# wkvong/multimodal-baby

Measured on AMD Instinct MI355X. Metric: image-text pairs/sec, CVCL ResNeXt+embed 224², bs256, 1/2/4/8 MI355X, higher is better.
Workload: dtype bf16; 1 GPU; C2 = BASELINE configs[1]: CVCL saycam_contrastive, frozen random-init ResNeXt-50 32x4d (BN train mode) + embedding mean-pool text encoder, E=512, L2-normalised, fixed tau 0.07, 224x224 frames + 3-word utterances; full step = fwd + InfoNCE + bwd(fc, embedding) + AdamW; per_gpu_batch=256, global_batch=256, negatives=local (single GPU), parallelism=dp1, trunk_streams=2

## Files before the change

multimodal-baby_amd/csrc/resnext.hip:

```cpp
#include <algorithm>
#include <array>
#include <cstdlib>
#include <type_traits>

#include "cvcl_common.h"

namespace {

constexpr int kMaxStatsRows = 1024;
constexpr size_t kTrunkAccLayer = (size_t)kBnAccRows * 2 * 2048;


__global__ __launch_bounds__(1024) void bn_finalize_kernel(const float* __restrict__ stats, int rows, double count,
                                                           const float* __restrict__ gamma, const float* __restrict__ beta,
                                                           float* __restrict__ running_mean, float* __restrict__ running_var,
                                                           int64_t* __restrict__ nbt, float momentum, float eps,
                                                           float* __restrict__ scale, float* __restrict__ shift, int C,
                                                           float* __restrict__ moments, int moments_ld,
                                                           const float* __restrict__ centre) {
    constexpr int NS = 64, NC = 16;
    __shared__ double ps[NS][NC], pq[NS][NC];
    const int c = threadIdx.x & (NC - 1), sl = threadIdx.x / NC, ch = blockIdx.x * NC + c;
    double s = 0.0, q = 0.0;
    if (ch < C) {
// ... 96 lines not shown
            q = fmaf(v, v, q);
        }
    }
    ps[sl][c] = s;
    pq[sl][c] = q;
    __syncthreads();
    if (sl == 0 && ch < C) {
        stats[((long)blockIdx.x * 2 + 0) * C + ch] = (ps[0][c] + ps[1][c]) + (ps[2][c] + ps[3][c]);
        stats[((long)blockIdx.x * 2 + 1) * C + ch] = (pq[0][c] + pq[1][c]) + (pq[2][c] + pq[3][c]);
    }
}

template <typename T>
__global__ void cast_kernel(const float* __restrict__ in, T* __restrict__ out, long n) {
    for (long i = (long)blockIdx.x * blockDim.x + threadIdx.x; i < n; i += (long)gridDim.x * blockDim.x)
        out[i] = ElemTraits<T>::from_f(in[i]);
}

__global__ void pack_stem_kernel(const float* __restrict__ w, bf16_t* __restrict__ out) {
    const int i = blockIdx.x * blockDim.x + threadIdx.x;
    if (i >= 4 * 6 * 16 * 32) return;
    const int k = i & 31, n = (i >> 5) & 15, ks = (i >> 9) % 6, nt = i / (6 * 512);
    const int r = 4 * ks + (k >> 3), kx = k & 7;
    float v = 0.f;
    if (r < 21 && kx < 7) {
        const int c = r / 7, ky = r % 7;
        v = w[((nt * 16 + n) * 3 + c) * 49 + ky * 7 + kx];
    }
    out[i] = (bf16_t)v;
}

__global__ void pack_gconv_kernel(const float* __restrict__ w, bf16_t* __restrict__ out, int C, int cg) {
    const int KS = cg == 32 ? 9 : 5;
    const long total = (long)(C / 16) * KS * 512;
    const long i = (long)blockIdx.x * blockDim.x + threadIdx.x;
    if (i >= total) return;
    const int k = (int)(i & 31), n = (int)((i >> 5) & 15), ks = (int)((i >> 9) % KS), unit = (int)(i / ((long)KS * 512));
    const int co = unit * 16 + n;
    float v = 0.f;
    if (cg == 32) {
        v = w[((long)co * 32 + k) * 9 + ks];
    } else {
        const int tap = 2 * ks + (k >> 4), ci_abs = unit * 16 + (k & 15);
        if (tap < 9 && ci_abs / cg == co / cg) v = w[((long)co * cg + (ci_abs % cg)) * 9 + tap];
    }
    out[i] = (bf16_t)v;
}

constexpr int STEM_TH = 4;
constexpr int STEM_ROWS = 2 * STEM_TH + 5;
constexpr int STEM_PITCH = 144;
constexpr int STEM_OPITCH = 144;

__global__ __launch_bounds__(256, 2) void stem_mfma_kernel(const float* __restrict__ x, const bf16_t* __restrict__ wp,
                                                        bf16_t* __restrict__ y, float* __restrict__ stats,
                                                        const float* __restrict__ centre, int B, int Hin, int Win) {
    extern __shared__ __attribute__((aligned(16))) char smem[];
    unsigned int* patch = (unsigned int*)smem;
    const int Ho = Hin / 2, Wo = Win / 2;
    const int bands = cvcl_div_up(Ho, STEM_TH);
    const int tid = threadIdx.x, lane = tid & 63, wave = tid >> 6;
    const int pix = lane & 15, kb = lane >> 4;

    bf16x8 wf[4][6];
#pragma unroll
    for (int nt = 0; nt < 4; ++nt)
#pragma unroll
        for (int ks = 0; ks < 6; ++ks)
            wf[nt][ks] = *reinterpret_cast<const bf16x8*>(wp + ((nt * 6 + ks) * 16 + pix) * 32 + kb * 8);

    f32x2 ssum[4][2], ssq[4][2];
#pragma unroll
    for (int a = 0; a < 4; ++a)
#pragma unroll
        for (int b = 0; b < 2; ++b) { ssum[a][b] = f32x2{0.f, 0.f}; ssq[a][b] = f32x2{0.f, 0.f}; }

    const int mtiles_per_row = cvcl_div_up(Wo, 16);
    const int wave_u = __builtin_amdgcn_readfirstlane(wave);
    int koff[6];
#pragma unroll
    for (int ks = 0; ks < 6; ++ks) {
        const int r = min(4 * ks + kb, 20);
        const int c = r / 7, ky = r - c * 7;
        koff[ks] = (c * STEM_ROWS + ky) * STEM_PITCH;
    }
    for (int i = tid; i < 3 * STEM_ROWS * STEM_PITCH; i += 256) patch[i] = 0u;
    char* wst = smem + 3 * STEM_ROWS * STEM_PITCH * 4 + wave * (16 * STEM_OPITCH);
    float* cen = reinterpret_cast<float*>(smem + 3 * STEM_ROWS * STEM_PITCH * 4 + 4 * 16 * STEM_OPITCH);
    if (tid < 64) cen[tid] = centre ? -centre[tid] : 0.f;
    const int bx = (gridDim.x & 7) == 0 ? (int)((blockIdx.x & 7) * (gridDim.x >> 3) + (blockIdx.x >> 3)) : (int)blockIdx.x;
    for (int item = bx; item < B * bands; item += gridDim.x) {
        const int b = item / bands, band = item - b * bands;
        const int oy0 = band * STEM_TH;
        __syncthreads();
        {
            constexpr int NROW = 3 * STEM_ROWS, NV = 5;
            const int vec_per_row = Win / 4, jl = min(lane, vec_per_row - 1);
#pragma unroll
            for (int half = 0; half < 2; ++half) {
                f32x4 v[NV];
#pragma unroll
                for (int i = 0; i < NV; ++i) {
                    const int r = min((half * NV + i) * 4 + wave_u, NROW - 1);
                    const int c = r / STEM_ROWS, iy = r - c * STEM_ROWS;
                    const int yin = min(max(2 * oy0 - 3 + iy, 0), Hin - 1);
                    v[i] = *reinterpret_cast<const f32x4*>(x + (((long)b * 3 + c) * Hin + yin) * Win + 4 * jl);
                }
#pragma unroll
                for (int i = 0; i < NV; ++i) {
                    const int r = (half * NV + i) * 4 + wave_u;
                    const int iy = r % STEM_ROWS, yin = 2 * oy0 - 3 + iy;
                    if (r < NROW && lane < vec_per_row) {
                        const bool ok = yin >= 0 && yin < Hin;
                        const unsigned u01 = ok ? round2(f32x2{v[i][0], v[i][1]}) : 0u, u23 = ok ? round2(f32x2{v[i][2], v[i][3]}) : 0u;
                        char* dst = reinterpret_cast<char*>(patch + r * STEM_PITCH) + 8 * lane + 6;
                        *reinterpret_cast<unsigned short*>(dst) = (unsigned short)u01;
                        *reinterpret_cast<unsigned*>(dst + 2) = (u01 >> 16) | (u23 << 16);
                        *reinterpret_cast<unsigned short*>(dst + 6) = (unsigned short)(u23 >> 16);
                    }
                }
            }
        }
        __syncthreads();
        int ty = 0, tx = wave_u;
        while (tx >= mtiles_per_row) { tx -= mtiles_per_row; ++ty; }
        while (ty < STEM_TH) {
            const int ox0 = tx * 16;
            const int oy = oy0 + ty, ox = ox0 + pix;
            f32x4 acc[4];
#pragma unroll
            for (int nt = 0; nt < 4; ++nt) acc[nt] = *reinterpret_cast<const f32x4*>(cen + nt * 16 + kb * 4);
            const unsigned int* row0 = patch + 2 * ty * STEM_PITCH + (ox < Wo ? ox : 0);
#pragma unroll
            for (int ks = 0; ks < 6; ++ks) {
                const unsigned int* src = row0 + koff[ks];
                u32x4 raw = {src[0], src[1], src[2], src[3]};
                const bf16x8 bfrag = __builtin_bit_cast(bf16x8, raw);
#pragma unroll
                for (int nt = 0; nt < 4; ++nt)
                    acc[nt] = __builtin_amdgcn_mfma_f32_16x16x32_bf16(wf[nt][ks], bfrag, acc[nt], 0, 0, 0);
            }
            const bool inside = oy < Ho && ox < Wo;
#pragma unroll
            for (int nt = 0; nt < 4; ++nt) {
                const u32x2 o = {round2(f32x2{acc[nt][0], acc[nt][1]}), round2(f32x2{acc[nt][2], acc[nt][3]})};
                *reinterpret_cast<u32x2*>(wst + pix * STEM_OPITCH + nt * 32 + kb * 8) = o;
                if (inside) {
#pragma unroll
                    for (int e = 0; e < 2; ++e) {
                        const f32x2 sv = widen2(o[e]);
                        ssum[nt][e] += sv;
                        ssq[nt][e] = __builtin_elementwise_fma(sv, sv, ssq[nt][e]);
                    }
                }
            }
            __builtin_amdgcn_wave_barrier();
            asm volatile("" ::: "memory");
            if (oy < Ho && y) {
                bf16_t* drow = y + (((long)b * Ho + oy) * Wo + ox0) * 64 + (lane & 7) * 8;
#pragma unroll
                for (int rd = 0; rd < 2; ++rd) {
                    const int px = (lane >> 3) + 8 * rd;
                    const u32x4 v = *reinterpret_cast<const u32x4*>(wst + px * STEM_OPITCH + (lane & 7) * 16);
                    if (ox0 + px < Wo) *reinterpret_cast<u32x4*>(drow + (long)px * 64) = v;
                }
            }
            __builtin_amdgcn_wave_barrier();
            asm volatile("" ::: "memory");
            tx += 4;
            while (tx >= mtiles_per_row) { tx -= mtiles_per_row; ++ty; }
        }
    }
    __syncthreads();
    float* red = (float*)smem;
#pragma unroll
    for (int nt = 0; nt < 4; ++nt)
#pragma unroll
        for (int e = 0; e < 4; ++e) {
            float s = ssum[nt][e >> 1][e & 1], q = ssq[nt][e >> 1][e & 1];
#pragma unroll
            for (int o = 1; o < 16; o <<= 1) { s += __shfl_xor(s, o, 64); q += __shfl_xor(q, o, 64); }
            if (pix == 0) {
                red[(wave * 2 + 0) * 64 + nt * 16 + kb * 4 + e] = s;
                red[(wave * 2 + 1) * 64 + nt * 16 + kb * 4 + e] = q;
            }
        }
    __syncthreads();
    if (tid < 128) {
        const int which = tid >> 6, c = tid & 63;
        const float v = (red[(0 * 2 + which) * 64 + c] + red[(1 * 2 + which) * 64 + c]) +
                        (red[(2 * 2 + which) * 64 + c] + red[(3 * 2 + which) * 64 + c]);
        stats[((long)blockIdx.x * 2 + which) * 64 + c] = v;
    }
}

constexpr int STEMP_TP = 2;
constexpr int STEMP_CR = 2 * STEMP_TP + 1;
constexpr int STEMP_ROWS = 2 * STEMP_CR + 5;
constexpr int STEMP_BW = 128;
constexpr int STEMP_BAND_BYTES = (STEMP_CR * STEMP_BW + 1) * 128;
__global__ __launch_bounds__(512, 1) void stem_pool_mfma_kernel(const float* __restrict__ x, const bf16_t* __restrict__ wp,
                                                                bf16_t* __restrict__ y, const float* __restrict__ scale,
                                                                const float* __restrict__ shift, const float* __restrict__ centre,
                                                                int B, int Hin, int Win) {
    extern __shared__ __attribute__((aligned(16))) char smem[];
    unsigned int* patch = (unsigned int*)smem;
    char* band = smem + 3 * STEMP_ROWS * STEM_PITCH * 4;
    float* cen = reinterpret_cast<float*>(band + STEMP_BAND_BYTES);
    const int Ho = Hin / 2, Wo = Win / 2;
    const int Hp = (Ho - 1) / 2 + 1, Wp = (Wo - 1) / 2 + 1;
    const int bands = cvcl_div_up(Hp, STEMP_TP);
    const int tid = threadIdx.x, lane = tid & 63;
    const int wave_u = __builtin_amdgcn_readfirstlane(tid >> 6);
    const int pix = lane & 15, kb = lane >> 4;

    bf16x8 wf[4][6];
#pragma unroll
    for (int nt = 0; nt < 4; ++nt)
#pragma unroll
        for (int ks = 0; ks < 6; ++ks)
            wf[nt][ks] = *reinterpret_cast<const bf16x8*>(wp + ((nt * 6 + ks) * 16 + pix) * 32 + kb * 8);
    const int mtiles_per_row = cvcl_div_up(Wo, 16);
    int koff[6];
#pragma unroll
    for (int ks = 0; ks < 6; ++ks) {
        const int r = min(4 * ks + kb, 20);
        const int c = r / 7, ky = r - c * 7;
        koff[ks] = (c * STEMP_ROWS + ky) * STEM_PITCH;
    }
    for (int i = tid; i < 3 * STEMP_ROWS * STEM_PITCH; i += 512) patch[i] = 0u;
    for (int i = tid; i < STEMP_CR * STEMP_BW * 32; i += 512) reinterpret_cast<unsigned*>(band)[i] = 0u;
    if (tid < 64) {
        cen[tid] = centre ? -centre[tid] : 0.f;
        cen[64 + tid] = scale[tid];
        cen[128 + tid] = shift[tid];
    }
    const int bx = (gridDim.x & 7) == 0 ? (int)((blockIdx.x & 7) * (gridDim.x >> 3) + (blockIdx.x >> 3)) : (int)blockIdx.x;
    for (int item = bx; item < B * bands; item += gridDim.x) {
        const int b = item / bands, bnd = item - b * bands;
        const int p0 = bnd * STEMP_TP;
        const int oy_first = 2 * p0 - 1;
        {
            constexpr int NROW = 3 * STEMP_ROWS, NV = (NROW + 15) / 16;
            const int vec_per_row = Win / 4, jl = min(lane, vec_per_row - 1);
#pragma unroll
            for (int half = 0; half < 2; ++half) {
                f32x4 v[NV];
#pragma unroll
                for (int i = 0; i < NV; ++i) {
                    const int r = min((half * NV + i) * 8 + wave_u, NROW - 1);
                    const int c = r / STEMP_ROWS, iy = r - c * STEMP_ROWS;
                    const int yin = min(max(2 * oy_first - 3 + iy, 0), Hin - 1);
                    v[i] = *reinterpret_cast<const f32x4*>(x + (((long)b * 3 + c) * Hin + yin) * Win + 4 * jl);
                }
#pragma unroll
                for (int i = 0; i < NV; ++i) {
                    const int r = (half * NV + i) * 8 + wave_u;
                    const int iy = r % STEMP_ROWS, yin = 2 * oy_first - 3 + iy;
                    if (r < NROW && lane < vec_per_row) {
                        const bool ok = yin >= 0 && yin < Hin;
                        const unsigned u01 = ok ? round2(f32x2{v[i][0], v[i][1]}) : 0u, u23 = ok ? round2(f32x2{v[i][2], v[i][3]}) : 0u;
                        char* dst = reinterpret_cast<char*>(patch + r * STEM_PITCH) + 8 * lane + 6;
                        *reinterpret_cast<unsigned short*>(dst) = (unsigned short)u01;
                        *reinterpret_cast<unsigned*>(dst + 2) = (u01 >> 16) | (u23 << 16);
                        *reinterpret_cast<unsigned short*>(dst + 6) = (unsigned short)(u23 >> 16);
                    }
                }
            }
        }
        __syncthreads();
        for (int t = wave_u; t < STEMP_CR * mtiles_per_row; t += 8) {
            const int ty = t / mtiles_per_row, tx = t - ty * mtiles_per_row;
            const int ox0 = tx * 16, ox = ox0 + pix;
            const int oy = oy_first + ty;
            char* brow = band + (ty * STEMP_BW + ox + 1) * 128 + kb * 8;
            if (oy < 0 || oy >= Ho) {
#pragma unroll
                for (int nt = 0; nt < 4; ++nt) *reinterpret_cast<u32x2*>(brow + nt * 32) = u32x2{0u, 0u};
                continue;
            }
            f32x4 acc[4];
#pragma unroll
            for (int nt = 0; nt < 4; ++nt) acc[nt] = *reinterpret_cast<const f32x4*>(cen + nt * 16 + kb * 4);
            const unsigned int* row0 = patch + 2 * ty * STEM_PITCH + (ox < Wo ? ox : 0);
#pragma unroll
            for (int ks = 0; ks < 6; ++ks) {
                const unsigned int* src = row0 + koff[ks];
                u32x4 raw = {src[0], src[1], src[2], src[3]};
                const bf16x8 bfrag = __builtin_bit_cast(bf16x8, raw);
#pragma unroll
                for (int nt = 0; nt < 4; ++nt)
                    acc[nt] = __builtin_amdgcn_mfma_f32_16x16x32_bf16(wf[nt][ks], bfrag, acc[nt], 0, 0, 0);
            }
            const bool inside = ox < Wo;
#pragma unroll
            for (int nt = 0; nt < 4; ++nt) {
                const u32x2 o = {round2(f32x2{acc[nt][0], acc[nt][1]}), round2(f32x2{acc[nt][2], acc[nt][3]})};
                const f32x4 sc4 = *reinterpret_cast<const f32x4*>(cen + 64 + nt * 16 + kb * 4);
                const f32x4 sh4 = *reinterpret_cast<const f32x4*>(cen + 128 + nt * 16 + kb * 4);
                const f32x2 r01 = widen2(o[0]), r23 = widen2(o[1]);
                const f32x2 v01 = {fmaxf(fmaf(r01[0], sc4[0], sh4[0]), 0.f), fmaxf(fmaf(r01[1], sc4[1], sh4[1]), 0.f)};
                const f32x2 v23 = {fmaxf(fmaf(r23[0], sc4[2], sh4[2]), 0.f), fmaxf(fmaf(r23[1], sc4[3], sh4[3]), 0.f)};
                *reinterpret_cast<u32x2*>(brow + nt * 32) = inside ? u32x2{round2(v01), round2(v23)} : u32x2{0u, 0u};
            }
        }
        __syncthreads();
        typedef unsigned short u16x8 __attribute__((ext_vector_type(8)));
        for (int u = tid; u < STEMP_TP * Wp * 8; u += 512) {
            const int c8 = u & 7, q = u >> 3;
            const int pr = q / Wp, pc = q - pr * Wp;
            if (p0 + pr >= Hp) continue;
            const char* src = band + ((2 * pr) * STEMP_BW + 2 * pc) * 128 + c8 * 16;
            u16x8 m = *reinterpret_cast<const u16x8*>(src);
#pragma unroll
            for (int dy = 0; dy < 3; ++dy)
#pragma unroll
                for (int dx = 0; dx < 3; ++dx) {
                    if (dy == 0 && dx == 0) continue;
                    m = __builtin_elementwise_max(m, *reinterpret_cast<const u16x8*>(src + (dy * STEMP_BW + dx) * 128));
                }
            *reinterpret_cast<u16x8*>(y + (((long)b * Hp + p0 + pr) * Wp + pc) * 64 + c8 * 8) = m;
        }
    }
}

__global__ __launch_bounds__(256) void stem_direct_f32_kernel(const float* __restrict__ x, const float* __restrict__ w,
                                                              float* __restrict__ y, const float* __restrict__ centre,
                                                              int B, int Hin, int Win) {
    const int Ho = Hin / 2, Wo = Win / 2;
    const long total = (long)B * Ho * Wo * 64;
    for (long i = (long)blockIdx.x * blockDim.x + threadIdx.x; i < total; i += (long)gridDim.x * blockDim.x) {
        const int co = (int)(i & 63);
        const long p = i >> 6;
        const int ox = (int)(p % Wo), oy = (int)((p / Wo) % Ho), b = (int)(p / ((long)Wo * Ho));
        float acc = centre ? -centre[co] : 0.f;
        for (int c = 0; c < 3; ++c)
            for (int ky = 0; ky < 7; ++ky) {
                const int yin = 2 * oy - 3 + ky;
                if (yin < 0 || yin >= Hin) continue;
                for (int kx = 0; kx < 7; ++kx) {
                    const int xin = 2 * ox - 3 + kx;
                    if (xin < 0 || xin >= Win) continue;
                    acc = fmaf(x[(((long)b * 3 + c) * Hin + yin) * Win + xin], w[((co * 3 + c) * 7 + ky) * 7 + kx], acc);
                }
            }
        y[i] = acc;
    }
}

__global__ __launch_bounds__(256) void stem_tiled_f32_kernel(const float* __restrict__ x, const float* __restrict__ w,
                                                             float* __restrict__ y, const float* __restrict__ centre,
                                                             int B, int Hin, int Win, int TH, int bands) {
    extern __shared__ __attribute__((aligned(16))) float smf[];
    const int Ho = Hin / 2, Wo = Win / 2;
    const int Wp = Win + 6, rows_in = 2 * TH + 5, plane = rows_in * Wp;
    float* ws = smf;
    float* cs = ws + 147 * 64;
    float* xs = cs + 64;
    const int tid = threadIdx.x, lane = tid & 63;
    const int wave = __builtin_amdgcn_readfirstlane(tid >> 6);
    for (int e = tid; e < 147 * 64; e += 256) {
        const int co = e / 147, tap = e - co * 147;
        ws[tap * 64 + co] = w[e];
    }
    if (tid < 64) cs[tid] = centre ? -centre[tid] : 0.f;
    for (int item = blockIdx.x; item < B * bands; item += gridDim.x) {
        const int b = item / bands, band = item - b * bands;
        const int oy0 = band * TH, iy0 = 2 * oy0 - 3;
        __syncthreads();
        for (int e = tid; e < 3 * plane; e += 256) {
            const int c = e / plane, r = e - c * plane, ry = r / Wp, rx = r - ry * Wp;
            const int yin = iy0 + ry, xin = rx - 3;
// ... 700 lines not shown
        if (kind == CVCL_PACK_GCONV3) {
            CVCL_CHECK_ARG(k == 3, "cvcl_pack_conv_weight: grouped conv must be 3x3");
            return cvcl_pack_split_conv(0, w_oihw, out, cout, cin_per_group, stream);
        }
        cvcl_set_error("cvcl_pack_conv_weight: unknown kind %d", kind);
        return CVCL_EINVAL;
    }
    if (dtype == CVCL_F32) {
        hipLaunchKernelGGL(cast_kernel<float>, dim3(cvcl_grid(n, 256, 4096)), dim3(256), 0, s, w_oihw, (float*)out, n);
    } else if (kind == CVCL_PACK_DENSE) {
        hipLaunchKernelGGL(cast_kernel<bf16_t>, dim3(cvcl_grid(n, 256, 4096)), dim3(256), 0, s, w_oihw, (bf16_t*)out, n);
    } else if (kind == CVCL_PACK_STEM7) {
        CVCL_CHECK_ARG(cout == 64 && cin_per_group == 3 && k == 7, "cvcl_pack_conv_weight: stem must be 64x3x7x7");
        hipLaunchKernelGGL(pack_stem_kernel, dim3(cvcl_div_up(4 * 6 * 512, 256)), dim3(256), 0, s, w_oihw, (bf16_t*)out);
    } else if (kind == CVCL_PACK_GCONV3) {
        CVCL_CHECK_ARG(k == 3 && (cin_per_group == 4 || cin_per_group == 8 || cin_per_group == 16 || cin_per_group == 32) &&
                           cout % 64 == 0, "cvcl_pack_conv_weight: unsupported grouped conv %d/%d", cout, cin_per_group);
        const long total = (long)(cout / 16) * (cin_per_group == 32 ? 9 : 5) * 512;
        hipLaunchKernelGGL(pack_gconv_kernel, dim3(cvcl_div_up(total, 256)), dim3(256), 0, s, w_oihw, (bf16_t*)out, cout,
                           cin_per_group);
    } else {
        cvcl_set_error("cvcl_pack_conv_weight: unknown kind %d", kind);
        return CVCL_EINVAL;
    }
    CVCL_LAUNCH_CHECK();
    return CVCL_OK;
}

static int stem_grid(int B, int Hin) {
    const int items = B * cvcl_div_up(Hin / 2, STEM_TH);
    return items < 512 ? items : 512;
}

extern "C" int cvcl_stem_conv_stats_rows(int dtype, int B, int H, int W) {
    if (!cvcl_dtype_trunk(dtype)) return 0;
    if (dtype == CVCL_F32X3) return cvcl_stem_split_stats_rows(B, H, W);
    if (dtype == CVCL_BF16) return stem_grid(B, H);
    return cvcl_col_stats_rows((long)B * (H / 2) * (W / 2));
}

extern "C" int cvcl_stem_conv7x7(int dtype, const float* x_nchw, const void* w_packed, void* y_nhwc, float* stats,
                                 int stats_rows, const float* centre, int B, int H, int W, void* stream) {
    CVCL_CHECK_DTYPE_TRUNK(dtype, "cvcl_stem_conv7x7");
    if (dtype == CVCL_F32X3)
        return cvcl_stem_split(x_nchw, w_packed, (float*)y_nhwc, stats, stats_rows, centre, B, H, W, stream);
    CVCL_CHECK_ARG(x_nchw && w_packed && (y_nhwc || (dtype == CVCL_BF16 && stats)) && B > 0 && H % 2 == 0 && W % 2 == 0,
                   "cvcl_stem_conv7x7: bad args");
    hipStream_t s = (hipStream_t)stream;
    if (dtype == CVCL_BF16) {
        CVCL_CHECK_ARG(W + 6 + 8 <= 2 * STEM_PITCH && W % 4 == 0 && W / 4 <= 64,
                       "cvcl_stem_conv7x7: width %d not supported by the staged patch", W);
        const int g = stem_grid(B, H);
        CVCL_CHECK_ARG(!stats || stats_rows >= g, "cvcl_stem_conv7x7: stats_rows %d < %d", stats_rows, g);
        const size_t lds = (size_t)3 * STEM_ROWS * STEM_PITCH * 4 + 4 * 16 * STEM_OPITCH + 64 * 4;
        float* st = stats;
        CVCL_CHECK_ARG(st, "cvcl_stem_conv7x7: the bf16 kernel always emits statistics; pass a buffer");
        CvclProfScope prof(stream, CVCL_K_STEM);
        hipLaunchKernelGGL(stem_mfma_kernel, dim3(g), dim3(256), lds, s, x_nchw, (const bf16_t*)w_packed, (bf16_t*)y_nhwc,
                           st, centre, B, H, W);
        CVCL_LAUNCH_CHECK();
        return CVCL_OK;
    }
    const long total = (long)B * (H / 2) * (W / 2) * 64;
    {
        CvclProfScope prof(stream, CVCL_K_STEM);
        const int Ho = H / 2;
        auto lds_of = [&](int th) { return (size_t)(147 * 64 + 64 + 3 * (2 * th + 5) * (W + 6)) * 4; };
        int TH = Ho < 8 ? Ho : 8;
        while (TH > 1 && lds_of(TH) > 150 * 1024) --TH;
        if (lds_of(TH) <= 150 * 1024) {
            static CvclLdsAttr attr;
            if (const int rc = cvcl_raise_lds_limit(attr, (const void*)stem_tiled_f32_kernel, 160 * 1024, "cvcl_stem_conv7x7")) return rc;
            attr.mark();
            const int bands = cvcl_div_up(Ho, TH);
            const long items = (long)B * bands;
            hipLaunchKernelGGL(stem_tiled_f32_kernel, dim3((unsigned)(items < 1024 ? items : 1024)), dim3(256), lds_of(TH), s, x_nchw,
                               (const float*)w_packed, (float*)y_nhwc, centre, B, H, W, TH, bands);
        } else {
            hipLaunchKernelGGL(stem_direct_f32_kernel, dim3(cvcl_grid(total, 256, 8192)), dim3(256), 0, s, x_nchw,
                               (const float*)w_packed, (float*)y_nhwc, centre, B, H, W);
        }
    }
    CVCL_LAUNCH_CHECK();
    if (stats) return cvcl_col_stats(CVCL_F32, y_nhwc, (long)B * (H / 2) * (W / 2), 64, stats, stats_rows, stream);
    return CVCL_OK;
}

extern "C" int cvcl_stem_pool_supported(int dtype, int H, int W) {
    return dtype == CVCL_BF16 && H % 2 == 0 && W % 4 == 0 && W / 4 <= 64 && W + 6 + 8 <= 2 * STEM_PITCH && W / 2 + 2 <= STEMP_BW;
}

extern "C" int cvcl_stem_pool(int dtype, const float* x_nchw, const void* w_packed, const float* scale, const float* shift,
                              const float* centre, void* y_nhwc, int B, int H, int W, void* stream) {
    CVCL_CHECK_DTYPE(dtype, "cvcl_stem_pool");
    CVCL_CHECK_ARG(x_nchw && w_packed && scale && shift && y_nhwc && B > 0, "cvcl_stem_pool: bad args");
    CVCL_CHECK_ARG(cvcl_stem_pool_supported(dtype, H, W), "cvcl_stem_pool: bf16 and a width <= %d only (got dtype %d, %d x %d)",
                   2 * (STEMP_BW - 2), dtype, H, W);
    const size_t lds = (size_t)3 * STEMP_ROWS * STEM_PITCH * 4 + (size_t)STEMP_BAND_BYTES + 3 * 64 * 4;
    static CvclLdsAttr attr;
    if (const int rc = cvcl_raise_lds_limit(attr, (const void*)stem_pool_mfma_kernel, (int)lds, "cvcl_stem_pool")) return rc;
    attr.mark();
    const int Hp = (H / 2 - 1) / 2 + 1;
    const int items = B * cvcl_div_up(Hp, STEMP_TP);
    int dev = 0, cus = 256;
    if (hipGetDevice(&dev) != hipSuccess || hipDeviceGetAttribute(&cus, hipDeviceAttributeMultiprocessorCount, dev) != hipSuccess || cus <= 0) cus = 256;
    const int grid = items < cus ? items : cus;
    CvclProfScope prof(stream, CVCL_K_STEM);
    hipLaunchKernelGGL(stem_pool_mfma_kernel, dim3(grid), dim3(512), lds, (hipStream_t)stream, x_nchw, (const bf16_t*)w_packed,
                       (bf16_t*)y_nhwc, scale, shift, centre, B, H, W);
    CVCL_LAUNCH_CHECK();
    return CVCL_OK;
}

extern "C" int cvcl_bn_relu_maxpool(int dtype, const void* x, const float* scale, const float* shift, void* y, int B,
                                    int H, int W, int C, void* stream) {
    CVCL_CHECK_DTYPE_TRUNK(dtype, "cvcl_bn_relu_maxpool");
    dtype = cvcl_storage_dtype(dtype);
    CVCL_CHECK_ARG(x && scale && shift && y && C % 8 == 0, "cvcl_bn_relu_maxpool: bad args");
    CvclProfScope prof(stream, CVCL_K_MAXPOOL);
    const int Ho = (H - 1) / 2 + 1, Wo = (W - 1) / 2 + 1;
    const long total = (long)B * ((Ho + POOL_ROWS - 1) / POOL_ROWS) * Wo * (C / 8);
    const int grid = cvcl_grid(total, 256, 8192);
    if (dtype == CVCL_F32)
        hipLaunchKernelGGL(bn_relu_maxpool_kernel<float>, dim3(grid), dim3(256), 0, (hipStream_t)stream,
                           (const float*)x, scale, shift, (float*)y, B, H, W, C);
    else
        hipLaunchKernelGGL(bn_relu_maxpool_kernel<bf16_t>, dim3(grid), dim3(256), 0, (hipStream_t)stream,
                           (const bf16_t*)x, scale, shift, (bf16_t*)y, B, H, W, C);
    CVCL_LAUNCH_CHECK();
    return CVCL_OK;
}

namespace {
struct GconvPlan { int TH, bands, rows_in, grid_x; size_t lds; };
GconvPlan gconv_plan(int B, int H, int W, int C, int stride) {
    GconvPlan g;
    const int Ho = (H - 1) / stride + 1, Wo = (W - 1) / stride + 1, Wp = W + 2;
    auto bytes = [&](int th) { return (size_t)(((th - 1) * stride + 3) * Wp + th * Wo) * GC_PIXB; };
    int TH = Ho;
    while (TH > 1 && (bytes(TH) > (size_t)52 * 1024 || ((TH - 1) * stride + 3) * Wp > 10 * 32 || TH * Wo > 128)) TH = (TH + 1) / 2;
    g.TH = TH;
    g.bands = cvcl_div_up(Ho, TH);
    g.rows_in = (TH - 1) * stride + 3;
    g.lds = bytes(TH);
    int per_cu = (int)((160 * 1024) / g.lds);
    const int reg_limit = (C / 32 == 32) ? 2 : 3;
    if (per_cu > reg_limit) per_cu = reg_limit;
    if (per_cu < 1) per_cu = 1;
    const int slabs = C / GC_CS;
    int gx = per_cu * 256 / slabs;
    if (gx < 1) gx = 1;
// ... 445 lines not shown
    }
    long long* acc = (training && dtype == CVCL_BF16) ? ws.acc : nullptr;
    if (acc && hipMemsetAsync(acc, 0, (size_t)n_layers * kAccBytes, (hipStream_t)stream) != hipSuccess) {
        cvcl_set_error("cvcl_resnext50_block_fwd: cannot clear the BatchNorm accumulators");
        return CVCL_ELAUNCH;
    }
    const BnLayers bn = {layers, ws.affine, nullptr, centres, acc};
    if (!training)
        for (int l = 0; l < n_layers; ++l)
            if (int rc = cvcl_bn_eval_affine(layers[l].gamma, layers[l].beta, layers[l].running_mean, layers[l].running_var, eps,
                                             bn.scale(l), bn.shift(l), bn.centre(l), block_layer_c(stage, l), stream)) return rc;
    const PassCtx ctx = {dtype, B, training, momentum, eps, ws.stats, ws.gram, stream};
    return bottleneck_fwd(ctx, block_geom(B, stage, first != 0, h, w, 0),
                          BlockBufs<char>{(char*)x_nhwc, (char*)out_nhwc, ws.R1, ws.R2, ws.R1, ws.RD}, bn);
}

static int resnext50_fwd_impl(int dtype, int B, int H, int W, int training, const float* x_nchw,
                              const cvcl_convbn_params* layers, int n_layers, void* workspace, size_t workspace_bytes,
                              void* layer4_out_nhwc, float* pooled, float momentum, float eps, float* moments,
                              const float* centres, void* stream) {
    CVCL_CHECK_DTYPE_TRUNK(dtype, "cvcl_resnext50_fwd");
    CVCL_CHECK_ARG(x_nchw && layers && workspace && layer4_out_nhwc && pooled, "cvcl_resnext50_fwd: null pointer");
    CVCL_CHECK_ARG(((uintptr_t)centres & 15) == 0, "cvcl_resnext50_fwd: centres must be 16-byte aligned");
    CVCL_CHECK_ARG(n_layers == kTrunkLayers, "cvcl_resnext50_fwd: expected 53 conv+bn layers, got %d", n_layers);
    CVCL_CHECK_ARG(B > 0 && H % 32 == 0 && W % 32 == 0, "cvcl_resnext50_fwd: H, W must be multiples of 32");
    const TrunkLayout ws(dtype, B, H, W, workspace);
    if (workspace_bytes < ws.bytes) {
        cvcl_set_error("cvcl_resnext50_fwd: workspace too small");
        return CVCL_EWORKSPACE;
    }
    long long* acc = (training && dtype == CVCL_BF16) ? ws.acc : nullptr;
    if (acc && hipMemsetAsync(acc, 0, kTrunkLayers * kAccBytes, (hipStream_t)stream) != hipSuccess) {
        cvcl_set_error("cvcl_resnext50_fwd: cannot clear the BatchNorm accumulators");
        return CVCL_ELAUNCH;
    }
    int rc;
    if (!training) {
        const EvalAffineAll t = trunk_table<EvalAffineAll>(layers);
        for (int i = 0; i < kTrunkLayers; ++i)
            CVCL_CHECK_ARG(t.gamma[i] && t.beta[i] && t.rm[i] && t.rv[i], "cvcl_resnext50_fwd: layer %d lacks BatchNorm tensors", i);
        CvclProfScope prof(stream, CVCL_K_BN_FINALIZE);
        static const bool centred = cvcl_env_on("CVCL_CENTRED_STORAGE");
        float* own = (!centres && centred && dtype == CVCL_BF16) ? ws.centres : nullptr;
        hipLaunchKernelGGL(bn_eval_affine_all_kernel, dim3(kTrunkLayers), dim3(256), 0, (hipStream_t)stream, t, eps, ws.affine, centres,
                           own);
        CVCL_LAUNCH_CHECK();
        if (own) centres = own;
    }
    const PassCtx ctx = {dtype, B, training, momentum, eps, ws.stats, ws.gram, stream};
    const BnLayers bn = {layers, ws.affine, moments, centres, acc};

    int h = H / 2, wd = W / 2;
    char* RAW = ws.buf[2];
    if ((rc = cvcl_stem_conv7x7(dtype, x_nchw, layers[0].w, RAW, ws.stats, kMaxStatsRows, centres, B, H, W, stream))) return rc;
    if ((rc = bn.finalize(ctx, 0, cvcl_stem_conv_stats_rows(dtype, B, H, W), (long)B * h * wd, 64))) return rc;
    if ((rc = cvcl_bn_relu_maxpool(dtype, RAW, bn.scale(0), bn.shift(0), ws.buf[0], B, h, wd, 64, stream))) return rc;
    h /= 2; wd /= 2;
    if ((rc = walk_blocks(B, h, wd, ws.buf, (char*)layer4_out_nhwc, [&](const BlockGeom& g, const BlockBufs<char>& io) {
             return bottleneck_fwd(ctx, g, io, bn.from(g.li));
         }))) return rc;
    return cvcl_avgpool(dtype, layer4_out_nhwc, pooled, B, h * wd, kMaxC, stream);
}

extern "C" int cvcl_resnext50_fwd(int dtype, int B, int H, int W, int training, const float* x_nchw,
                                  const cvcl_convbn_params* layers, int n_layers, void* workspace, size_t workspace_bytes,
                                  void* layer4_out_nhwc, float* pooled, float momentum, float eps, const float* centres,
                                  void* stream) {
    return resnext50_fwd_impl(dtype, B, H, W, training, x_nchw, layers, n_layers, workspace, workspace_bytes, layer4_out_nhwc, pooled,
                              momentum, eps, nullptr, centres, stream);
}

extern "C" size_t cvcl_resnext50_moments_floats(void) { return (size_t)kTrunkLayers * kAffStride; }

extern "C" int cvcl_resnext50_fwd_deferred_stats(int dtype, int B, int H, int W, const float* x_nchw,
                                                 const cvcl_convbn_params* layers, int n_layers, void* workspace,
                                                 size_t workspace_bytes, void* layer4_out_nhwc, float* pooled, float eps,
                                                 float* moments, const float* centres, void* stream) {
    CVCL_CHECK_ARG(moments, "cvcl_resnext50_fwd_deferred_stats: moments is NULL");
    return resnext50_fwd_impl(dtype, B, H, W, 1, x_nchw, layers, n_layers, workspace, workspace_bytes, layer4_out_nhwc, pooled,
                              0.f, eps, moments, centres, stream);
}

extern "C" int cvcl_resnext50_apply_moments(const cvcl_convbn_params* layers, int n_layers, const float* moments, float momentum,
                                            void* stream) {
    CVCL_CHECK_ARG(layers && moments && n_layers == kTrunkLayers,
                   "cvcl_resnext50_apply_moments: expected 53 conv+bn layers and their moments");
    const ApplyMomentsAll t = trunk_table<ApplyMomentsAll>(layers);
    for (int i = 0; i < kTrunkLayers; ++i)
        CVCL_CHECK_ARG(t.rm[i] && t.rv[i], "cvcl_resnext50_apply_moments: layer %d lacks running statistics", i);
    CvclProfScope prof(stream, CVCL_K_BN_FINALIZE);
    hipLaunchKernelGGL(bn_apply_moments_kernel, dim3(kTrunkLayers), dim3(256), 0, (hipStream_t)stream, t, moments, momentum);
    CVCL_LAUNCH_CHECK();
    return CVCL_OK;
}

namespace {
int group_slices(int T, long rows_g, int C) {
    long s = 2048 / ((long)T * (C / 64));
    if (s > 64) s = 64;
    if (s > rows_g / 64) s = rows_g / 64;
    return s < 1 ? 1 : (int)s;
}
size_t group_part_floats(int T) { return (size_t)128 * std::max<size_t>(2048, (size_t)32 * T); }
bool grouped_dtype(int dtype) { return dtype == CVCL_F32 || dtype == CVCL_F32X3; }

struct GroupedLayout {
    float *buf[5], *part, *aff[4];
    size_t bytes;
    GroupedLayout(int B, int H, int W, int T, void* base = nullptr) {
// ... 98 lines not shown
```

Measured before the change: 52500 pairs/s.

## Double-buffer stem input patches and prefetch next band; swizzle pool band LDS

The stem conv and fused stem+pool kernels now keep two LDS patch buffers and issue global loads for the next band before computing the current one, depositing them afterwards so load latency overlaps MFMA work. A stats-only variant of the stem kernel (no output store) is templated out. The pool band layout is XOR-swizzled to cut LDS bank conflicts, and the centre, scale and shift constants are held in registers. Eval mode routes through the fused stem+pool path. The cost is more LDS per block and more registers, which may lower occupancy.

New measurement: 52400 pairs/s. Within noise of the previous version (-0.2%).

```diff
diff --git a/multimodal-baby_amd/csrc/resnext.hip b/multimodal-baby_amd/csrc/resnext.hip
--- a/multimodal-baby_amd/csrc/resnext.hip
+++ b/multimodal-baby_amd/csrc/resnext.hip
@@ -172,10 +172,44 @@
 constexpr int STEM_PITCH = 144;
 constexpr int STEM_OPITCH = 144;
 
+template <int ROWS, int WAVES>
+struct StemRows {
+    static constexpr int NROW = 3 * ROWS, NS = (NROW + WAVES - 1) / WAVES;
+    f32x4 v[NS];
+    __device__ __forceinline__ void request(const float* __restrict__ x, int b, int y0, int Hin, int Win, int wave_u, int lane) {
+        const int jl = min(lane, Win / 4 - 1);
+#pragma unroll
+        for (int i = 0; i < NS; ++i) {
+            const int r = min(i * WAVES + wave_u, NROW - 1);
+            const int c = r / ROWS, iy = r - c * ROWS;
+            const int yin = min(max(y0 + iy, 0), Hin - 1);
+            v[i] = *reinterpret_cast<const f32x4*>(x + (((long)b * 3 + c) * Hin + yin) * Win + 4 * jl);
+        }
+    }
+    static __device__ __forceinline__ void arrived() { __builtin_amdgcn_s_waitcnt(0x0F70); }
+    __device__ __forceinline__ void deposit(unsigned int* patch, int y0, int Hin, int Win, int wave_u, int lane) const {
+#pragma unroll
+        for (int i = 0; i < NS; ++i) {
+            const int r = i * WAVES + wave_u;
+            const int iy = r % ROWS, yin = y0 + iy;
+            if (r < NROW && lane < Win / 4) {
+                const bool ok = yin >= 0 && yin < Hin;
+                const unsigned u01 = ok ? round2(f32x2{v[i][0], v[i][1]}) : 0u, u23 = ok ? round2(f32x2{v[i][2], v[i][3]}) : 0u;
+                char* dst = reinterpret_cast<char*>(patch + r * STEM_PITCH) + 8 * lane + 6;
+                *reinterpret_cast<unsigned short*>(dst) = (unsigned short)u01;
+                *reinterpret_cast<unsigned*>(dst + 2) = (u01 >> 16) | (u23 << 16);
+                *reinterpret_cast<unsigned short*>(dst + 6) = (unsigned short)(u23 >> 16);
+            }
+        }
+    }
+};
+
+template <bool STORE>
 __global__ __launch_bounds__(256, 2) void stem_mfma_kernel(const float* __restrict__ x, const bf16_t* __restrict__ wp,
                                                         bf16_t* __restrict__ y, float* __restrict__ stats,
                                                         const float* __restrict__ centre, int B, int Hin, int Win) {
     extern __shared__ __attribute__((aligned(16))) char smem[];
+    constexpr int PATCH_DW = 3 * STEM_ROWS * STEM_PITCH, NPATCH = STORE ? 1 : 2;
     unsigned int* patch = (unsigned int*)smem;
     const int Ho = Hin / 2, Wo = Win / 2;
     const int bands = cvcl_div_up(Ho, STEM_TH);
@@ -204,16 +238,41 @@
         const int c = r / 7, ky = r - c * 7;
         koff[ks] = (c * STEM_ROWS + ky) * STEM_PITCH;
     }
-    for (int i = tid; i < 3 * STEM_ROWS * STEM_PITCH; i += 256) patch[i] = 0u;
-    char* wst = smem + 3 * STEM_ROWS * STEM_PITCH * 4 + wave * (16 * STEM_OPITCH);
-    float* cen = reinterpret_cast<float*>(smem + 3 * STEM_ROWS * STEM_PITCH * 4 + 4 * 16 * STEM_OPITCH);
-    if (tid < 64) cen[tid] = centre ? -centre[tid] : 0.f;
+    for (int i = tid; i < NPATCH * PATCH_DW; i += 256) patch[i] = 0u;
+    char* wst = smem + NPATCH * PATCH_DW * 4 + wave * (16 * STEM_OPITCH);
+    float* cen = reinterpret_cast<float*>(smem + NPATCH * PATCH_DW * 4 + (STORE ? 4 * 16 * STEM_OPITCH : 0));
+    if (STORE && tid < 64) cen[tid] = centre ? -centre[tid] : 0.f;
+    f32x4 negc[4];
+    if constexpr (!STORE) {
+#pragma unroll
+        for (int nt = 0; nt < 4; ++nt)
+#pragma unroll
+            for (int e = 0; e < 4; ++e) negc[nt][e] = centre ? -centre[nt * 16 + kb * 4 + e] : 0.f;
+    }
     const int bx = (gridDim.x & 7) == 0 ? (int)((blockIdx.x & 7) * (gridDim.x >> 3) + (blockIdx.x >> 3)) : (int)blockIdx.x;
-    for (int item = bx; item < B * bands; item += gridDim.x) {
+    const int total = B * bands;
+    StemRows<STEM_ROWS, 4> nxt;
+    int pbuf = 0;
+    if constexpr (!STORE) {
+        const int b0 = bx / bands, y0 = 2 * (bx - b0 * bands) * STEM_TH - 3;
+        if (bx < total) nxt.request(x, b0, y0, Hin, Win, wave_u, lane);
+        __syncthreads();
+        nxt.arrived();
+        if (bx < total) nxt.deposit(patch, y0, Hin, Win, wave_u, lane);
+    }
+    for (int item = bx; item < total; item += gridDim.x) {
         const int b = item / bands, band = item - b * bands;
         const int oy0 = band * STEM_TH;
-        __syncthreads();
-        {
+        const int nitem = item + (int)gridDim.x;
+        const bool more = !STORE && nitem < total;
+        const int nb = nitem / bands, ny0 = 2 * (nitem - nb * bands) * STEM_TH - 3;
+        if constexpr (!STORE) {
+            if (more) nxt.request(x, nb, ny0, Hin, Win, wave_u, lane);
+            __syncthreads();
+            patch = (unsigned int*)smem + pbuf * PATCH_DW;
+        }
+        if constexpr (STORE) __syncthreads();
+        if constexpr (STORE) {
             constexpr int NROW = 3 * STEM_ROWS, NV = 5;
             const int vec_per_row = Win / 4, jl = min(lane, vec_per_row - 1);
 #pragma unroll
@@ -240,8 +299,8 @@
                     }
                 }
             }
-        }
-        __syncthreads();
+            __syncthreads();
+        }
         int ty = 0, tx = wave_u;
         while (tx >= mtiles_per_row) { tx -= mtiles_per_row; ++ty; }
         while (ty < STEM_TH) {
@@ -249,7 +308,7 @@
             const int oy = oy0 + ty, ox = ox0 + pix;
             f32x4 acc[4];
 #pragma unroll
-            for (int nt = 0; nt < 4; ++nt) acc[nt] = *reinterpret_cast<const f32x4*>(cen + nt * 16 + kb * 4);
+            for (int nt = 0; nt < 4; ++nt) acc[nt] = STORE ? *reinterpret_cast<const f32x4*>(cen + nt * 16 + kb * 4) : negc[nt];
             const unsigned int* row0 = patch + 2 * ty * STEM_PITCH + (ox < Wo ? ox : 0);
 #pragma unroll
             for (int ks = 0; ks < 6; ++ks) {
@@ -264,7 +323,7 @@
 #pragma unroll
             for (int nt = 0; nt < 4; ++nt) {
                 const u32x2 o = {round2(f32x2{acc[nt][0], acc[nt][1]}), round2(f32x2{acc[nt][2], acc[nt][3]})};
-                *reinterpret_cast<u32x2*>(wst + pix * STEM_OPITCH + nt * 32 + kb * 8) = o;
+                if constexpr (STORE) *reinterpret_cast<u32x2*>(wst + pix * STEM_OPITCH + nt * 32 + kb * 8) = o;
                 if (inside) {
 #pragma unroll
                     for (int e = 0; e < 2; ++e) {
@@ -274,21 +333,28 @@
                     }
                 }
             }
-            __builtin_amdgcn_wave_barrier();
-            asm volatile("" ::: "memory");
-            if (oy < Ho && y) {
-                bf16_t* drow = y + (((long)b * Ho + oy) * Wo + ox0) * 64 + (lane & 7) * 8;
-#pragma unroll
-                for (int rd = 0; rd < 2; ++rd) {
-                    const int px = (lane >> 3) + 8 * rd;
-                    const u32x4 v = *reinterpret_cast<const u32x4*>(wst + px * STEM_OPITCH + (lane & 7) * 16);
-                    if (ox0 + px < Wo) *reinterpret_cast<u32x4*>(drow + (long)px * 64) = v;
+            if constexpr (STORE) {
+                __builtin_amdgcn_wave_barrier();
+                asm volatile("" ::: "memory");
+                if (oy < Ho) {
+                    bf16_t* drow = y + (((long)b * Ho + oy) * Wo + ox0) * 64 + (lane & 7) * 8;
+#pragma unroll
+                    for (int rd = 0; rd < 2; ++rd) {
+                        const int px = (lane >> 3) + 8 * rd;
+                        const u32x4 v = *reinterpret_cast<const u32x4*>(wst + px * STEM_OPITCH + (lane & 7) * 16);
+                        if (ox0 + px < Wo) *reinterpret_cast<u32x4*>(drow + (long)px * 64) = v;
+                    }
                 }
-            }
-            __builtin_amdgcn_wave_barrier();
-            asm volatile("" ::: "memory");
+                __builtin_amdgcn_wave_barrier();
+                asm volatile("" ::: "memory");
+            }
             tx += 4;
             while (tx >= mtiles_per_row) { tx -= mtiles_per_row; ++ty; }
+        }
+        if constexpr (!STORE) {
+            nxt.arrived();
+            if (more) nxt.deposit((unsigned int*)smem + (pbuf ^ 1) * PATCH_DW, ny0, Hin, Win, wave_u, lane);
+            pbuf ^= 1;
         }
     }
     __syncthreads();
@@ -319,14 +385,15 @@
 constexpr int STEMP_ROWS = 2 * STEMP_CR + 5;
 constexpr int STEMP_BW = 128;
 constexpr int STEMP_BAND_BYTES = (STEMP_CR * STEMP_BW + 1) * 128;
+constexpr int STEMP_PATCHES = 2;
 __global__ __launch_bounds__(512, 1) void stem_pool_mfma_kernel(const float* __restrict__ x, const bf16_t* __restrict__ wp,
                                                                 bf16_t* __restrict__ y, const float* __restrict__ scale,
                                                                 const float* __restrict__ shift, const float* __restrict__ centre,
                                                                 int B, int Hin, int Win) {
     extern __shared__ __attribute__((aligned(16))) char smem[];
-    unsigned int* patch = (unsigned int*)smem;
-    char* band = smem + 3 * STEMP_ROWS * STEM_PITCH * 4;
-    float* cen = reinterpret_cast<float*>(band + STEMP_BAND_BYTES);
+    constexpr int PATCH_DW = 3 * STEMP_ROWS * STEM_PITCH;
+    unsigned int* patches = (unsigned int*)smem;
+    char* band = smem + STEMP_PATCHES * PATCH_DW * 4;
     const int Ho = Hin / 2, Wo = Win / 2;
     const int Hp = (Ho - 1) / 2 + 1, Wp = (Wo - 1) / 2 + 1;
     const int bands = cvcl_div_up(Hp, STEMP_TP);
@@ -348,60 +415,53 @@
         const int c = r / 7, ky = r - c * 7;
         koff[ks] = (c * STEMP_ROWS + ky) * STEM_PITCH;
     }
-    for (int i = tid; i < 3 * STEMP_ROWS * STEM_PITCH; i += 512) patch[i] = 0u;
+    for (int i = tid; i < STEMP_PATCHES * PATCH_DW; i += 512) patches[i] = 0u;
     for (int i = tid; i < STEMP_CR * STEMP_BW * 32; i += 512) reinterpret_cast<unsigned*>(band)[i] = 0u;
-    if (tid < 64) {
-        cen[tid] = centre ? -centre[tid] : 0.f;
-        cen[64 + tid] = scale[tid];
-        cen[128 + tid] = shift[tid];
-    }
+    f32x4 negc[4], sc[4], sh[4];
+#pragma unroll
+    for (int nt = 0; nt < 4; ++nt)
+#pragma unroll
+        for (int e = 0; e < 4; ++e) {
+            const int ch = nt * 16 + kb * 4 + e;
+            negc[nt][e] = centre ? -centre[ch] : 0.f;
+            sc[nt][e] = scale[ch];
+            sh[nt][e] = shift[ch];
+        }
     const int bx = (gridDim.x & 7) == 0 ? (int)((blockIdx.x & 7) * (gridDim.x >> 3) + (blockIdx.x >> 3)) : (int)blockIdx.x;
-    for (int item = bx; item < B * bands; item += gridDim.x) {
+    const int total = B * bands;
+    StemRows<STEMP_ROWS, 8> nxt;
+    int pbuf = 0;
+    {
+        const int b0 = bx / bands, y0 = 2 * (2 * (bx - b0 * bands) * STEMP_TP - 1) - 3;
+        if (bx < total) nxt.request(x, b0, y0, Hin, Win, wave_u, lane);
+        __syncthreads();
+        nxt.arrived();
+        if (bx < total) nxt.deposit(patches, y0, Hin, Win, wave_u, lane);
+    }
+    for (int item = bx; item < total; item += gridDim.x) {
         const int b = item / bands, bnd = item - b * bands;
         const int p0 = bnd * STEMP_TP;
         const int oy_first = 2 * p0 - 1;
-        {
-            constexpr int NROW = 3 * STEMP_ROWS, NV = (NROW + 15) / 16;
-            const int vec_per_row = Win / 4, jl = min(lane, vec_per_row - 1);
-#pragma unroll
-            for (int half = 0; half < 2; ++half) {
-                f32x4 v[NV];
-#pragma unroll
-                for (int i = 0; i < NV; ++i) {
-                    const int r = min((half * NV + i) * 8 + wave_u, NROW - 1);
-                    const int c = r / STEMP_ROWS, iy = r - c * STEMP_ROWS;
-                    const int yin = min(max(2 * oy_first - 3 + iy, 0), Hin - 1);
-                    v[i] = *reinterpret_cast<const f32x4*>(x + (((long)b * 3 + c) * Hin + yin) * Win + 4 * jl);
-                }
-#pragma unroll
-                for (int i = 0; i < NV; ++i) {
-                    const int r = (half * NV + i) * 8 + wave_u;
-                    const int iy = r % STEMP_ROWS, yin = 2 * oy_first - 3 + iy;
-                    if (r < NROW && lane < vec_per_row) {
-                        const bool ok = yin >= 0 && yin < Hin;
-                        const unsigned u01 = ok ? round2(f32x2{v[i][0], v[i][1]}) : 0u, u23 = ok ? round2(f32x2{v[i][2], v[i][3]}) : 0u;
-                        char* dst = reinterpret_cast<char*>(patch + r * STEM_PITCH) + 8 * lane + 6;
-                        *reinterpret_cast<unsigned short*>(dst) = (unsigned short)u01;
-                        *reinterpret_cast<unsigned*>(dst + 2) = (u01 >> 16) | (u23 << 16);
-                        *reinterpret_cast<unsigned short*>(dst + 6) = (unsigned short)(u23 >> 16);
-                    }
-                }
-            }
-        }
+        const int nitem = item + (int)gridDim.x;
+        const bool more = nitem < total;
+        const int nb = nitem / bands, ny0 = 2 * (2 * (nitem - nb * bands) * STEMP_TP - 1) - 3;
+        if (more) nxt.request(x, nb, ny0, Hin, Win, wave_u, lane);
         __syncthreads();
+        const unsigned int* patch = patches + pbuf * PATCH_DW;
         for (int t = wave_u; t < STEMP_CR * mtiles_per_row; t += 8) {
             const int ty = t / mtiles_per_row, tx = t - ty * mtiles_per_row;
             const int ox0 = tx * 16, ox = ox0 + pix;
             const int oy = oy_first + ty;
-            char* brow = band + (ty * STEMP_BW + ox + 1) * 128 + kb * 8;
+            char* bpix = band + (ty * STEMP_BW + ox + 1) * 128 + (kb & 1) * 8;
+            const int bsw = (kb >> 1) ^ ((ox + 1) & 7);
             if (oy < 0 || oy >= Ho) {
 #pragma unroll
-                for (int nt = 0; nt < 4; ++nt) *reinterpret_cast<u32x2*>(brow + nt * 32) = u32x2{0u, 0u};
+                for (int nt = 0; nt < 4; ++nt) *reinterpret_cast<u32x2*>(bpix + ((2 * nt) ^ bsw) * 16) = u32x2{0u, 0u};
                 continue;
             }
             f32x4 acc[4];
 #pragma unroll
-            for (int nt = 0; nt < 4; ++nt) acc[nt] = *reinterpret_cast<const f32x4*>(cen + nt * 16 + kb * 4);
+            for (int nt = 0; nt < 4; ++nt) acc[nt] = negc[nt];
             const unsigned int* row0 = patch + 2 * ty * STEM_PITCH + (ox < Wo ? ox : 0);
 #pragma unroll
             for (int ks = 0; ks < 6; ++ks) {
@@ -416,28 +476,30 @@
 #pragma unroll
             for (int nt = 0; nt < 4; ++nt) {
                 const u32x2 o = {round2(f32x2{acc[nt][0], acc[nt][1]}), round2(f32x2{acc[nt][2], acc[nt][3]})};
-                const f32x4 sc4 = *reinterpret_cast<const f32x4*>(cen + 64 + nt * 16 + kb * 4);
-                const f32x4 sh4 = *reinterpret_cast<const f32x4*>(cen + 128 + nt * 16 + kb * 4);
+                const f32x4 sc4 = sc[nt], sh4 = sh[nt];
                 const f32x2 r01 = widen2(o[0]), r23 = widen2(o[1]);
                 const f32x2 v01 = {fmaxf(fmaf(r01[0], sc4[0], sh4[0]), 0.f), fmaxf(fmaf(r01[1], sc4[1], sh4[1]), 0.f)};
                 const f32x2 v23 = {fmaxf(fmaf(r23[0], sc4[2], sh4[2]), 0.f), fmaxf(fmaf(r23[1], sc4[3], sh4[3]), 0.f)};
-                *reinterpret_cast<u32x2*>(brow + nt * 32) = inside ? u32x2{round2(v01), round2(v23)} : u32x2{0u, 0u};
-            }
-        }
+                *reinterpret_cast<u32x2*>(bpix + ((2 * nt) ^ bsw) * 16) = inside ? u32x2{round2(v01), round2(v23)} : u32x2{0u, 0u};
+            }
+        }
+        nxt.arrived();
+        if (more) nxt.deposit(patches + (pbuf ^ 1) * PATCH_DW, ny0, Hin, Win, wave_u, lane);
+        pbuf ^= 1;
         __syncthreads();
         typedef unsigned short u16x8 __attribute__((ext_vector_type(8)));
         for (int u = tid; u < STEMP_TP * Wp * 8; u += 512) {
             const int c8 = u & 7, q = u >> 3;
             const int pr = q / Wp, pc = q - pr * Wp;
             if (p0 + pr >= Hp) continue;
-            const char* src = band + ((2 * pr) * STEMP_BW + 2 * pc) * 128 + c8 * 16;
-            u16x8 m = *reinterpret_cast<const u16x8*>(src);
+            const char* src = band + ((2 * pr) * STEMP_BW + 2 * pc) * 128;
+            u16x8 m = u16x8{0, 0, 0, 0, 0, 0, 0, 0};
 #pragma unroll
             for (int dy = 0; dy < 3; ++dy)
 #pragma unroll
                 for (int dx = 0; dx < 3; ++dx) {
-                    if (dy == 0 && dx == 0) continue;
-                    m = __builtin_elementwise_max(m, *reinterpret_cast<const u16x8*>(src + (dy * STEMP_BW + dx) * 128));
+                    const int slot = c8 ^ ((2 * pc + dx) & 7);
+                    m = __builtin_elementwise_max(m, *reinterpret_cast<const u16x8*>(src + (dy * STEMP_BW + dx) * 128 + slot * 16));
                 }
             *reinterpret_cast<u16x8*>(y + (((long)b * Hp + p0 + pr) * Wp + pc) * 64 + c8 * 8) = m;
         }
@@ -1244,12 +1306,16 @@
                        "cvcl_stem_conv7x7: width %d not supported by the staged patch", W);
         const int g = stem_grid(B, H);
         CVCL_CHECK_ARG(!stats || stats_rows >= g, "cvcl_stem_conv7x7: stats_rows %d < %d", stats_rows, g);
-        const size_t lds = (size_t)3 * STEM_ROWS * STEM_PITCH * 4 + 4 * 16 * STEM_OPITCH + 64 * 4;
+        const size_t patch = (size_t)3 * STEM_ROWS * STEM_PITCH * 4;
         float* st = stats;
         CVCL_CHECK_ARG(st, "cvcl_stem_conv7x7: the bf16 kernel always emits statistics; pass a buffer");
         CvclProfScope prof(stream, CVCL_K_STEM);
-        hipLaunchKernelGGL(stem_mfma_kernel, dim3(g), dim3(256), lds, s, x_nchw, (const bf16_t*)w_packed, (bf16_t*)y_nhwc,
-                           st, centre, B, H, W);
+        if (y_nhwc)
+            hipLaunchKernelGGL(stem_mfma_kernel<true>, dim3(g), dim3(256), patch + 4 * 16 * STEM_OPITCH + 64 * 4, s, x_nchw,
+                               (const bf16_t*)w_packed, (bf16_t*)y_nhwc, st, centre, B, H, W);
+        else
+            hipLaunchKernelGGL(stem_mfma_kernel<false>, dim3(g), dim3(256), 2 * patch + 64 * 4, s, x_nchw, (const bf16_t*)w_packed,
+                               (bf16_t*)nullptr, st, centre, B, H, W);
         CVCL_LAUNCH_CHECK();
         return CVCL_OK;
     }
@@ -1288,7 +1354,7 @@
     CVCL_CHECK_ARG(x_nchw && w_packed && scale && shift && y_nhwc && B > 0, "cvcl_stem_pool: bad args");
     CVCL_CHECK_ARG(cvcl_stem_pool_supported(dtype, H, W), "cvcl_stem_pool: bf16 and a width <= %d only (got dtype %d, %d x %d)",
                    2 * (STEMP_BW - 2), dtype, H, W);
-    const size_t lds = (size_t)3 * STEMP_ROWS * STEM_PITCH * 4 + (size_t)STEMP_BAND_BYTES + 3 * 64 * 4;
+    const size_t lds = (size_t)STEMP_PATCHES * 3 * STEMP_ROWS * STEM_PITCH * 4 + (size_t)STEMP_BAND_BYTES;
     static CvclLdsAttr attr;
     if (const int rc = cvcl_raise_lds_limit(attr, (const void*)stem_pool_mfma_kernel, (int)lds, "cvcl_stem_pool")) return rc;
     attr.mark();
@@ -1840,9 +1906,13 @@
 
     int h = H / 2, wd = W / 2;
     char* RAW = ws.buf[2];
-    if ((rc = cvcl_stem_conv7x7(dtype, x_nchw, layers[0].w, RAW, ws.stats, kMaxStatsRows, centres, B, H, W, stream))) return rc;
-    if ((rc = bn.finalize(ctx, 0, cvcl_stem_conv_stats_rows(dtype, B, H, W), (long)B * h * wd, 64))) return rc;
-    if ((rc = cvcl_bn_relu_maxpool(dtype, RAW, bn.scale(0), bn.shift(0), ws.buf[0], B, h, wd, 64, stream))) return rc;
+    if (!training && cvcl_stem_pool_supported(dtype, H, W)) {
+        if ((rc = cvcl_stem_pool(dtype, x_nchw, layers[0].w, bn.scale(0), bn.shift(0), centres, ws.buf[0], B, H, W, stream))) return rc;
+    } else {
+        if ((rc = cvcl_stem_conv7x7(dtype, x_nchw, layers[0].w, RAW, ws.stats, kMaxStatsRows, centres, B, H, W, stream))) return rc;
+        if ((rc = bn.finalize(ctx, 0, cvcl_stem_conv_stats_rows(dtype, B, H, W), (long)B * h * wd, 64))) return rc;
+        if ((rc = cvcl_bn_relu_maxpool(dtype, RAW, bn.scale(0), bn.shift(0), ws.buf[0], B, h, wd, 64, stream))) return rc;
+    }
     h /= 2; wd /= 2;
     if ((rc = walk_blocks(B, h, wd, ws.buf, (char*)layer4_out_nhwc, [&](const BlockGeom& g, const BlockBufs<char>& io) {
              return bottleneck_fwd(ctx, g, io, bn.from(g.li));
```
